# MatteoBattilana/CUDAVideoStream

Measured on AMD Instinct MI355X. Metric: 1920×1080 RGB24 frames/sec (diff+threshold+pack); achieved HBM GB/s vs peak, higher is better.
Workload: dtype u8

## Files before the change

### cudavideostream_amd/csrc/core.hip

```cpp
#include <cmath>
#include <cstdio>
#include <cstdlib>
#include <cstring>
#include <new>
#include <string>
#include <vector>

#include "../../include/mi355diff.h"
#include "cwire_common.h"

using namespace mi355;

static inline size_t code_chunks(size_t max_batch) { return (max_batch + 2) / 3 + 1; }

namespace {

thread_local std::string g_err;

int fail(int code, const char *what, hipError_t e = hipSuccess) {
    char buf[512];
    if (e != hipSuccess)
        snprintf(buf, sizeof buf, "%s: %s (%s)", what, hipGetErrorName(e), hipGetErrorString(e));
    else
        snprintf(buf, sizeof buf, "%s", what);
    g_err = buf;
    return code;
}

// ... 2 lines not shown
        hipError_t _e = (expr);                                   \
        if (_e != hipSuccess) return fail(MI355_ERR_HIP, #expr, _e); \
    } while (0)

}

struct mi355_core {
    mi355_config cfg{};
    int device = 0;
    uint32_t n = 0;
    uint32_t ntiles = 0;
    hipStream_t own_stream = nullptr;
    hipStream_t stream = nullptr;

    uint8_t *state = nullptr, *in = nullptr, *aux = nullptr, *vis = nullptr;
    uint4 *rec = nullptr, *meta = nullptr;
    uint32_t *codes = nullptr;
    uint32_t *groff = nullptr, *totals = nullptr;
    uint64_t scan_epoch = 0;
    uint32_t *offsets = nullptr;
    int32_t *one_xs = nullptr;
    uint8_t *one_diff = nullptr;
    int32_t *hist = nullptr, *thr = nullptr;
    uint32_t *red_bounds = nullptr;
    uint32_t *cw_cnt = nullptr;
    uint4 *cw_items = nullptr;
    uint32_t *cw_esc = nullptr;
    CwaFrame *cwa_ftab = nullptr;
    uint4 *cwa_chunk = nullptr;
    uint4 *cwa_dir = nullptr;
    uint8_t *gray1 = nullptr;
// ... 11 lines not shown

    static constexpr int kMaxSlots = 8;
    struct Slot {
        uint8_t *d_in = nullptr, *d_vis = nullptr;
        uint32_t *h_count = nullptr;
        hipEvent_t uploaded = nullptr, painted = nullptr, packed = nullptr, shown = nullptr;
        bool has_vis = false;
        int64_t ticket = -1;
    };
    Slot slots[kMaxSlots];
    int nslots = 0;
    int64_t next_ticket = 0;
    hipStream_t up_stream = nullptr, down_stream = nullptr;

    struct LogSet {
        uint4 *rec = nullptr, *meta = nullptr;
        uint32_t *codes = nullptr, *groff = nullptr, *totals = nullptr;
        hipEvent_t packed = nullptr, expanded = nullptr;
        bool in_use = false;
    };
    static constexpr int kSets = 2;
    LogSet set[kSets];
    int flip = 0;
    hipStream_t side = nullptr;
    hipEvent_t side_done = nullptr;
    bool pipeline_ok = true;
    int median_rows = 0;
    uint32_t cu_count = 0;
    hipStream_t main2 = nullptr;
    hipEvent_t packed2[kSets] = {};
    static constexpr uint32_t kDensePct = 40;
// ... 116 lines not shown
}

int need_red_bounds(mi355_core *c) {
    if (c->red_bounds || c->n == 0) return MI355_OK;
    return dev_alloc(c, &c->red_bounds, (size_t)c->cfg.max_batch * red_bounds_per_frame(c->n));
}

int setup_pipeline(mi355_core *c) {
    if (c->side || !c->pipeline_ok) return MI355_OK;
    const size_t T = (size_t)c->cfg.max_batch, W = c->ntiles;
    mi355_core::LogSet &s0 = c->set[0], &s1 = c->set[1];
    s0.rec = c->rec; s0.codes = c->codes; s0.meta = c->meta; s0.groff = c->groff; s0.totals = c->totals;
    bool ok = true;
    ok = ok && hipMalloc((void **)&s1.rec, T * W * 1024) == hipSuccess;
    ok = ok && hipMalloc((void **)&s1.codes, code_chunks(T) * W * 1024) == hipSuccess;
    ok = ok && hipMalloc((void **)&s1.meta, T * W * 16) == hipSuccess;
    ok = ok && hipMalloc((void **)&s1.groff, T * expand_groups(c->ntiles) * 16) == hipSuccess;
    ok = ok && hipMalloc((void **)&s1.totals, (2 * T + 2) * sizeof(uint32_t)) == hipSuccess;
    ok = ok && hipMemsetAsync(s1.totals, 0, (2 * T + 2) * sizeof(uint32_t), c->stream) == hipSuccess &&
         hipStreamSynchronize(c->stream) == hipSuccess;
    ok = ok && make_stream(c, &c->side) == hipSuccess;
    ok = ok && make_stream(c, &c->main2) == hipSuccess;
    for (int i = 0; i < mi355_core::kSets && ok; i++) {
        const unsigned flags = hipEventDisableTiming | hipEventReleaseToDevice;
        ok = hipEventCreateWithFlags(&c->set[i].packed, flags) == hipSuccess &&
             hipEventCreateWithFlags(&c->set[i].expanded, flags) == hipSuccess &&
             hipEventCreateWithFlags(&c->packed2[i], flags) == hipSuccess &&
             hipEventCreateWithFlags(&c->fork[i], flags) == hipSuccess;
    }
    if (!ok) {
        (void)hipGetLastError();
        void *ptrs[] = {s1.rec, s1.codes, s1.meta, s1.groff, s1.totals};
        for (void *p : ptrs) if (p) (void)hipFree(p);
        s1.rec = nullptr; s1.meta = nullptr; s1.codes = s1.groff = s1.totals = nullptr;
        if (c->side) { (void)hipStreamDestroy(c->side); c->side = nullptr; }
        if (c->main2) { (void)hipStreamDestroy(c->main2); c->main2 = nullptr; }
        for (int i = 0; i < mi355_core::kSets; i++) {
            hipEvent_t *evs[] = {&c->set[i].packed, &c->set[i].expanded, &c->packed2[i], &c->fork[i]};
            for (hipEvent_t *e : evs) if (*e) { (void)hipEventDestroy(*e); *e = nullptr; }
        }
        c->pipeline_ok = false;
        return MI355_OK;
    }
    c->workspace += T * W * 1024 + code_chunks(T) * W * 1024 + T * W * 16 + T * expand_groups(c->ntiles) * 16 + (2 * T + 2) * 4;
    return MI355_OK;
}

struct CwireOut {
    uint64_t *frame_pos;
    uint8_t *cwire;
    uint64_t capacity;
};

CwireDirectArgs cwire_args(mi355_core *c, const CwireOut *cw, const uint32_t *d_offsets, uint32_t ntiles) {
    CwireDirectArgs x{};
    x.x.offsets = d_offsets;
    x.x.ntiles = ntiles;
    x.items = c->cw_items;
    x.esc = c->cw_esc;
// ... 54 lines not shown
    a.cur = (const uint8_t *)d_cur;
    a.prev = (const uint8_t *)d_prev;
    a.state = c->state;
    a.stride = stride;
    a.n = c->n;
    a.nframes = nframes;
    a.thr = c->cfg.threshold;
    a.ntiles = c->ntiles;
    a.tile_begin = 0;
    a.tile_end = c->ntiles;
    a.rec = ls.rec;
    a.codes = ls.codes;
    a.codes_bytes = (uint32_t)(code_chunks((size_t)c->cfg.max_batch) * c->ntiles * 1024u);
    a.meta = ls.meta;
    a.rec_bytes = (uint32_t)((size_t)c->cfg.max_batch * c->ntiles * 1024u);
    a.meta_bytes = (uint32_t)((size_t)c->cfg.max_batch * c->ntiles * 16u);
    const bool aligned = (((uintptr_t)d_cur | (uintptr_t)d_prev | stride) & 15u) == 0 && 3 * (uint64_t)stride + c->n < (1ull << 32);
    bool pair_once = false;
    if (pair) {
        const int64_t d = (int64_t)((intptr_t)d_prev - (intptr_t)d_cur), st = (int64_t)stride, T = nframes;
        bool shared = false;
        const int64_t k0 = d / st;
        for (int64_t k = k0 - 1; k <= k0 + 1; k++)
            if (k > -T && k < T && (d - k * st < 0 ? k * st - d : d - k * st) < (int64_t)c->n) shared = true;
        pair_once = !shared;
    }
    const uint32_t k1_blocks = 4u * c->cu_count;
    const bool split = pipelined && c->main2 && c->ntiles >= 64;
    if (split) {
        const uint32_t cut = (c->ntiles / 2) & ~3u;
        uint32_t blocks0 = 0, blocks1 = 0;
// ... 81 lines not shown
    if (!cfg || !out) return fail(MI355_ERR_INVALID, "null argument");
    *out = nullptr;
    if (cfg->width < 0 || cfg->height < 0) return fail(MI355_ERR_INVALID, "negative frame size");
    if (cfg->threshold < 0 || cfg->threshold > 255) return fail(MI355_ERR_INVALID, "threshold outside 0..255");
    if (cfg->max_batch < 1) return fail(MI355_ERR_INVALID, "max_batch < 1");
    if (cfg->visualizer < 0 || cfg->visualizer > 5) return fail(MI355_ERR_INVALID, "unknown visualizer");
    if (cfg->flags & ~MI355_FLAG_OWN_QUEUES) return fail(MI355_ERR_INVALID, "flags: unknown bit (MI355_FLAG_OWN_QUEUES is the only flag of this version of the library)");
    const uint64_t n64 = 3ull * (uint64_t)cfg->width * (uint64_t)cfg->height;
    if (n64 >= (1ull << 31)) return fail(MI355_ERR_INVALID, "frame larger than 2 GiB");
    {
        const uint64_t tiles = (n64 + kTileBytes - 1) / kTileBytes, mb = (uint64_t)cfg->max_batch;
        const uint64_t chunks = mb > code_chunks((size_t)mb) ? mb : (uint64_t)code_chunks((size_t)mb);
        if (tiles * kTileBytes * chunks >= (1ull << 32))
            return fail(MI355_ERR_INVALID, "max_batch * frame bytes must stay below 2^32");
    }

    int ndev = 0;
    hipError_t e = hipGetDeviceCount(&ndev);
    if (e != hipSuccess || ndev <= 0)
        return fail(MI355_ERR_HIP, "no HIP device available (libmi355diff has no CPU fallback)", e);
    mi355_core *c = new (std::nothrow) mi355_core;
    if (!c) return fail(MI355_ERR_INVALID, "out of host memory");
    c->cfg = *cfg;
    if (const char *v = getenv("MI355_PIPELINE")) c->pipeline_ok = v[0] != '0';
    if (cfg->device >= 0) c->device = cfg->device;
    else if ((e = hipGetDevice(&c->device)) != hipSuccess) { delete c; return fail(MI355_ERR_HIP, "hipGetDevice", e); }
    if (c->device >= ndev) { delete c; return fail(MI355_ERR_INVALID, "device ordinal out of range"); }

    c->n = (uint32_t)n64;
    c->ntiles = (c->n + kTileBytes - 1) / kTileBytes;
// ... 2 lines not shown
        if (hipGetDeviceProperties(&prop, c->device) == hipSuccess && prop.multiProcessorCount > 0) c->cu_count = (uint32_t)prop.multiProcessorCount;
    }
    const size_t T = (size_t)cfg->max_batch, W = c->ntiles, N = c->n;

    int rc = use_device(c);
    if (!rc) { e = make_stream(c, &c->own_stream); if (e != hipSuccess) rc = fail(MI355_ERR_HIP, "hipStreamCreate", e); }
    c->stream = c->own_stream;
    for (int i = 0; i < mi355_core::kEvRing * mi355_core::kEvPer && !rc; i++) { e = hipEventCreateWithFlags(&c->ev[i / mi355_core::kEvPer][i % mi355_core::kEvPer], hipEventDisableSystemFence); if (e != hipSuccess) rc = fail(MI355_ERR_HIP, "hipEventCreate", e); }
    if (!rc && (e = init_gray_table()) != hipSuccess) rc = fail(MI355_ERR_HIP, "init_gray_table", e);
    if (!rc) rc = dev_alloc(c, &c->state, N + 16);
    if (!rc) rc = dev_alloc(c, &c->in, N + 16);
    if (!rc) rc = dev_alloc(c, &c->aux, N + 16);
    if (!rc) rc = dev_alloc(c, &c->vis, N + 16);
    if (!rc) rc = dev_alloc(c, &c->rec, T * W * 64);
    if (!rc) rc = dev_alloc(c, &c->codes, code_chunks(T) * W * 256);
    if (!rc) rc = dev_alloc(c, &c->meta, T * W);
    if (!rc) rc = dev_alloc(c, &c->groff, T * expand_groups(c->ntiles) * 4);
    if (!rc) rc = dev_alloc(c, &c->totals, 2 * T + 2);
    if (!rc) { e = hipMemsetAsync(c->totals, 0, (2 * T + 2) * sizeof(uint32_t), c->own_stream); if (e != hipSuccess) rc = fail(MI355_ERR_HIP, "hipMemset", e); }
    if (!rc) rc = dev_alloc(c, &c->offsets, T + 1);
    if (!rc) rc = dev_alloc(c, &c->cw_cnt, (size_t)kCwireSlots);
    if (!rc) rc = dev_alloc(c, &c->cw_items, T * cwire_items_per_frame(c->ntiles));
    if (!rc) rc = dev_alloc(c, &c->cw_esc, T);
    if (!rc) rc = dev_alloc(c, &c->cwa_ftab, T);
    if (!rc) rc = dev_alloc(c, &c->cwa_chunk, T * cwa_chunks(c->n));
    if (!rc) rc = dev_alloc(c, &c->cwa_dir, T * cwa_tiles(c->n));
    if (!rc) rc = dev_alloc(c, &c->one_xs, N + 4);
    if (!rc) rc = dev_alloc(c, &c->one_diff, N + 16);
    if (!rc) rc = dev_alloc(c, &c->hist, 256 * T);
    if (!rc) rc = dev_alloc(c, &c->thr, T);
    if (!rc) rc = dev_alloc(c, &c->k9, 9);
// ... 985 lines not shown
```

### cudavideostream_amd/csrc/diff_pack.hip

```cpp
#include <cstdio>
#include <vector>

#include "cwire_common.h"
#include "pack_common.h"

namespace mi355 {

constexpr int kStreamPrefetch = 4;
template <bool PAIR>
struct PrefetchOf { static constexpr int value = PAIR ? 2 : kStreamPrefetch; };
static_assert(kStreamPrefetch % 2 == 0, "frames are processed in pairs");

typedef uint32_t u32x4 __attribute__((ext_vector_type(4)));
constexpr uint32_t kRsrcWord3 = 0x00020000u;
constexpr uint32_t kOOB = 0xFFFFFFFFu;

__device__ __forceinline__ __amdgpu_buffer_rsrc_t make_rsrc(const void *p, uint32_t bytes) {
    return __builtin_amdgcn_make_buffer_rsrc(const_cast<void *>(p), 0, (int)bytes, (int)kRsrcWord3);
}

struct LogOut {
    __amdgpu_buffer_rsrc_t codes, recs, meta;
};

template <bool HIGH>
__device__ __forceinline__ void compare_step(const uint4 c, uint4 &s, ThrConst tc, uint32_t (&dm)[4], uint32_t &m16) {
    const uint32_t cw[4] = {c.x, c.y, c.z, c.w};
    uint32_t sw[4] = {s.x, s.y, s.z, s.w};
// ... 1 lines not shown
#pragma unroll
    for (int k = 0; k < 4; k++) {
        uint32_t x;
        fh[k] = dword_flags<HIGH>(cw[k], sw[k], tc, x);
        const uint32_t mask = __builtin_amdgcn_perm(0u, 0u, fh[k]);
        dm[k] = bytes_sub_from_x(cw[k], sw[k], x, tc.h) & mask;
        sw[k] = bitop3<(TA & TC) | (TB & ~TC)>(cw[k], sw[k], mask);
    }
    s = make_uint4(sw[0], sw[1], sw[2], sw[3]);
    const uint32_t lo = __builtin_amdgcn_udot4(fh[1], tc.w1, __builtin_amdgcn_udot4(fh[0], tc.w0, 0u, false), false);
    const uint32_t hi = __builtin_amdgcn_udot4(fh[3], tc.w1, __builtin_amdgcn_udot4(fh[2], tc.w0, 0u, false), false);
    m16 = (lo + (hi << 8)) >> 7;
}

struct LogPos {
    uint32_t ptrC, roomC, ptrM, roomM;
};

__device__ __forceinline__ uint32_t emit_step(const uint32_t (&dm)[4], uint32_t m16, const LogOut &lg, LogPos &lp,
                                              uint32_t jump, uint32_t lane24, uint32_t &pc, uint32_t &pm) {
    const bool cand = m16 != 0u;
    const bool multi = (m16 & (m16 - 1u)) != 0u;
    const uint64_t bc = __ballot(cand), bm = __ballot(multi);
    const uint32_t rankC = __builtin_amdgcn_mbcnt_hi((uint32_t)(bc >> 32), __builtin_amdgcn_mbcnt_lo((uint32_t)bc, 0u));
    const uint32_t rankM = __builtin_amdgcn_mbcnt_hi((uint32_t)(bm >> 32), __builtin_amdgcn_mbcnt_lo((uint32_t)bm, 0u));
    const uint32_t nc = (uint32_t)__builtin_popcountll(bc), nm = (uint32_t)__builtin_popcountll(bm);
    pc = lp.ptrC;
    pm = lp.ptrM;
    if (nc == 0u) return 0u;
    if (nm > lp.roomM) { lp.ptrM += lp.roomM * 16u + jump; lp.roomM = 64u; }
    pm = lp.ptrM;
    if (nm == 64u) {
        const u32x4 v = {dm[0], dm[1], dm[2], dm[3]};
        __builtin_amdgcn_raw_buffer_store_b128(v, lg.recs, pm + rankM * 16u, 0, 0);
        lp.ptrM += 64u * 16u;
        lp.roomM -= 64u;
        return 64u | (64u << 16);
    }
    if (nc > lp.roomC) { lp.ptrC += lp.roomC * 4u + jump; lp.roomC = 256u; }
    pc = lp.ptrC;
    const uint32_t one = __builtin_amdgcn_sad_u8((dm[0] | dm[1]) | (dm[2] | dm[3]), 0u, 0u);
    const uint32_t code = m16 | ((multi ? rankM : one) << 16) | lane24;
    __builtin_amdgcn_raw_buffer_store_b32(code, lg.codes, cand ? pc + rankC * 4u : kOOB, 0, 0);
    const u32x4 v = {dm[0], dm[1], dm[2], dm[3]};
    __builtin_amdgcn_raw_buffer_store_b128(v, lg.recs, multi ? pm + rankM * 16u : kOOB, 0, 0);
    lp.ptrC += nc * 4u;
    lp.roomC -= nc;
    lp.ptrM += nm * 16u;
    lp.roomM -= nm;
    return nc | (nm << 16);
}

template <bool PAIR, bool FAST>
struct Group {
    static constexpr int kPrefetch = PrefetchOf<PAIR>::value;
    uint4 c[kPrefetch];
    uint4 p[kPrefetch];

    template <bool ONCE>
    __device__ __forceinline__ void load_desc(__amdgpu_buffer_rsrc_t cur, __amdgpu_buffer_rsrc_t prev, const uint32_t (&voff)[kPrefetch]) {
#pragma unroll
        for (int d = 0; d < kPrefetch; d++) {
            const u32x4 v = __builtin_amdgcn_raw_buffer_load_b128(cur, voff[d], 0, ONCE ? 2 : 0);
            c[d] = make_uint4(v.x, v.y, v.z, v.w);
            if (PAIR) {
// ... 11 lines not shown
            const bool in = t0 + d <= last;
            const uint8_t *cb = uniform_ptr(in ? cur0 + (size_t)d * a.stride : cur_last);
            c[d] = load16<FAST, !PAIR>(cb + byte_off, valid);
            if (PAIR) {
                const uint8_t *pb = uniform_ptr(in ? prev0 + (size_t)d * a.stride : prev_last);
                p[d] = load16<FAST>(pb + byte_off, valid);
            }
        }
    }
};

template <bool PAIR, bool FAST, bool HIGH>
__device__ __forceinline__ void pack_group(const PackArgs &a, const Group<PAIR, FAST> &g, int t0, uint4 &st,
                                           LogPos &lp, uint32_t tile, ThrConst tc, int lane, const LogOut &lg) {
    constexpr int kPrefetch = PrefetchOf<PAIR>::value;
    uint4 meta = make_uint4(0, 0, 0, 0);
    const uint32_t lane24 = ((uint32_t)lane << 24) | (tile << 30);
    const uint32_t jump = (a.ntiles - 1u) * 1024u;
#pragma unroll
    for (int d = 0; d < kPrefetch; d += 2) {
        const int t = t0 + d;
        if (t >= a.nframes) break;
        const bool two = t + 1 < a.nframes;
        uint32_t dm0[4], m0, m1 = 0, pc0, pm0, pc1 = 0, pm1 = 0;
        if (PAIR) st = g.p[d];
        compare_step<HIGH>(g.c[d], st, tc, dm0, m0);
        const uint32_t c0 = emit_step(dm0, m0, lg, lp, jump, lane24, pc0, pm0);
        uint32_t c1 = 0;
        if (two) {
            if (PAIR) st = g.p[d + 1];
            uint32_t dm1[4];
            compare_step<HIGH>(g.c[d + 1], st, tc, dm1, m1);
            c1 = emit_step(dm1, m1, lg, lp, jump, lane24, pc1, pm1);
        }
        const uint32_t both = (uint32_t)__builtin_popcount(m0) | ((uint32_t)__builtin_popcount(m1) << 16);
        const uint32_t tot = (uint32_t)__builtin_amdgcn_readlane(wave_inclusive_scan((int)both), 63);
        write_lane(meta.x, pc0, d);
        write_lane(meta.y, pm0, d);
        write_lane(meta.z, tot & 0xffffu, d);
        write_lane(meta.w, c0, d);
        write_lane(meta.x, pc1, d + 1);
        write_lane(meta.y, pm1, d + 1);
        write_lane(meta.z, tot >> 16, d + 1);
        write_lane(meta.w, c1, d + 1);
    }
    const uint32_t moff = (__umul24((uint32_t)t0 + (uint32_t)lane, a.ntiles) + tile) * 16u;
    const u32x4 mv = {meta.x, meta.y, meta.z, meta.w};
    __builtin_amdgcn_raw_buffer_store_b128(mv, lg.meta, (lane < kPrefetch && t0 + lane < a.nframes) ? moff : kOOB, 0, 0);
}

template <bool PAIR, bool FAST, bool HIGH, bool ONCE>
__device__ __forceinline__ void pack_tile(const PackArgs &a, uint32_t tile, uint32_t byte_off,
                                          int valid, int lane) {
    const int T = a.nframes;
    const ThrConst tc = make_thr((uint32_t)a.thr);
    const LogOut lg{make_rsrc(a.codes, a.codes_bytes), make_rsrc(a.rec, a.rec_bytes), make_rsrc(a.meta, a.meta_bytes)};

    uint4 st = make_uint4(0, 0, 0, 0);
    if (!PAIR) st = load16<FAST>(a.state + byte_off, valid);

    Group<PAIR, FAST> ga, gb;
    LogPos lp{tile * 1024u, 256u, tile * 1024u, 64u};
    constexpr int kPrefetch = PrefetchOf<PAIR>::value;
    const size_t gstep = (size_t)kPrefetch * a.stride;
    if (FAST) {
        uint32_t voff[kPrefetch];
#pragma unroll
        for (int d = 0; d < kPrefetch; d++) voff[d] = byte_off + (uint32_t)d * (uint32_t)a.stride;
        const uint8_t *cb = a.cur, *pb = a.prev;
        int64_t left = (int64_t)(T - 1) * (int64_t)a.stride + (int64_t)a.n;
        auto desc = [&](const uint8_t *base) {
            const uint32_t bytes = left <= 0 ? 0u : (left > 0xffffffffll ? 0xffffffffu : (uint32_t)left);
            return make_rsrc(base, bytes);
        };
        ga.template load_desc<ONCE>(desc(cb), desc(pb), voff);
        for (int t0 = 0;;) {
            cb += gstep; if (PAIR) pb += gstep; left -= (int64_t)gstep;
// ... 87 lines not shown
        for (int w = 0; w < NW; w++) {
            const uint32_t x = lds[w];
            lds[w] = acc;
            acc += x;
        }
        lds[NW] = acc;
    }
    __syncthreads();
    const uint32_t r = lds[wave] + incl - v;
    block_total = lds[NW];
    __syncthreads();
    return r;
}

constexpr uint32_t kXTiles = 64;
constexpr uint32_t kScanChunk = 1024;
constexpr uint32_t kScanDepth = 24;

__device__ __forceinline__ void publish_total(uint64_t *slot, uint32_t total, uint64_t epoch) {
    __hip_atomic_store(slot, (uint64_t)total | (epoch << kTotalBits), __ATOMIC_RELAXED, __HIP_MEMORY_SCOPE_AGENT);
}
__device__ __forceinline__ uint32_t read_total(const uint64_t *slot, uint64_t epoch) {
    uint64_t v;
    do v = __hip_atomic_load(slot, __ATOMIC_RELAXED, __HIP_MEMORY_SCOPE_AGENT);
    while ((v >> kTotalBits) != epoch);
    return (uint32_t)v & ((1u << kTotalBits) - 1u);
}

__global__ __launch_bounds__(256) void k_scan_groups(const uint4 *meta, uint32_t *roff, uint64_t *totals,
                                                     uint32_t ntiles, uint32_t ngroups, uint32_t *ticket,
                                                     uint64_t epoch, uint32_t *offsets, uint64_t *note) {
    static_assert(kXTiles == 64, "one wave reduces one group");
    __builtin_amdgcn_s_setprio(3);
    __shared__ uint32_t s_sum[kScanChunk];
    __shared__ uint32_t s_part[kScanChunk][3];
    __shared__ uint32_t s_scan[5];
    const uint32_t lane = threadIdx.x & 63, wave = threadIdx.x >> 6;
    const size_t row = (size_t)blockIdx.x * ntiles;
    uint32_t *out = roff + (size_t)blockIdx.x * ngroups * 4u;
    uint32_t carry = 0;
    for (uint32_t g0 = 0; g0 < ngroups; g0 += kScanChunk) {
        const uint32_t gn = min(kScanChunk, ngroups - g0);
        for (uint32_t g = wave * kScanDepth; g < gn; g += 4u * kScanDepth) {
            uint32_t z[kScanDepth];
#pragma unroll
            for (uint32_t k = 0; k < kScanDepth; k++) {
                const uint32_t tile = (g0 + g + k) * kXTiles + lane;
                z[k] = meta[row + min(tile, ntiles - 1u)].z;
            }
#pragma unroll
            for (uint32_t k = 0; k < kScanDepth; k++) {
                const uint32_t tile = (g0 + g + k) * kXTiles + lane;
                if (g + k >= gn || tile >= ntiles) z[k] = 0u;
                const uint32_t incl = (uint32_t)wave_inclusive_scan((int)z[k]);
                if (g + k < gn) {
                    if (lane == 63) s_sum[g + k] = incl;
                    if ((lane & 15u) == 15u && lane < 48u) s_part[g + k][lane >> 4] = incl;
                }
            }
        }
        __syncthreads();
        uint32_t v[4], sum = 0;
#pragma unroll
        for (uint32_t i = 0; i < 4; i++) {
            const uint32_t idx = threadIdx.x * 4 + i;
            v[i] = idx < gn ? s_sum[idx] : 0u;
            sum += v[i];
        }
        uint32_t total;
        uint32_t acc = carry + block_exclusive_scan<4>(sum, s_scan, total);
#pragma unroll
        for (uint32_t i = 0; i < 4; i++) {
            const uint32_t idx = threadIdx.x * 4 + i;
            if (idx < gn)
                *reinterpret_cast<uint4 *>(out + 4 * (size_t)(g0 + idx)) =
                    make_uint4(acc, acc + s_part[idx][0], acc + s_part[idx][1], acc + s_part[idx][2]);
            acc += v[i];
        }
        carry += total;
        __syncthreads();
    }
    __shared__ uint32_t s_is_last;
    if (threadIdx.x == 0) {
        publish_total(&totals[blockIdx.x], carry, epoch);
        s_is_last = __hip_atomic_fetch_add(ticket, 1u, __ATOMIC_RELAXED, __HIP_MEMORY_SCOPE_AGENT) == gridDim.x - 1;
    }
    __syncthreads();
    if (!s_is_last) return;
    const uint32_t nframes = gridDim.x;
    carry = 0;
    for (uint32_t base = 0; base < nframes; base += 256) {
        const uint32_t t = base + threadIdx.x;
        const uint32_t v = t < nframes ? read_total(&totals[t], epoch) : 0u;
        uint32_t total;
        const uint32_t ex = block_exclusive_scan<4>(v, s_scan, total);
        if (t < nframes) offsets[t] = carry + ex;
        carry += total;
    }
    if (threadIdx.x == 0) {
        offsets[nframes] = carry;
        __hip_atomic_store(ticket, 0u, __ATOMIC_RELAXED, __HIP_MEMORY_SCOPE_AGENT);
        if (note) __hip_atomic_store(note, (uint64_t)carry | ((uint64_t)nframes << 32), __ATOMIC_RELAXED, __HIP_MEMORY_SCOPE_SYSTEM);
    }
}

uint32_t expand_groups(uint32_t ntiles) { return (ntiles + kXTiles - 1) / kXTiles; }

hipError_t launch_scan(const uint4 *meta, uint32_t *roff, uint64_t *totals, uint32_t ntiles,
                       int nframes, uint32_t *offsets, uint32_t *ticket, uint64_t epoch, uint64_t *note, hipStream_t s) {
    hipLaunchKernelGGL(k_scan_groups, dim3(nframes), dim3(256), 0, s, meta, roff, totals, ntiles,
                       expand_groups(ntiles), ticket, epoch, offsets, note);
    return hipGetLastError();
}

__device__ __forceinline__ void store_u32_unaligned(uint8_t *p, uint32_t v) { __builtin_memcpy(p, &v, 4); }

__device__ __forceinline__ void lds_handoff() {
    __builtin_amdgcn_fence(__ATOMIC_ACQ_REL, "wavefront");
    __builtin_amdgcn_wave_barrier();
}

typedef uint32_t u32x4a4 __attribute__((ext_vector_type(4), aligned(4)));
typedef uint32_t u32x4a1 __attribute__((ext_vector_type(4), aligned(1)));
typedef uint32_t u32a1 __attribute__((aligned(1)));
template <bool BYTE_ALIGNED>
__device__ __forceinline__ void store_out4(uint8_t *p, uint32_t x, uint32_t y, uint32_t z, uint32_t w) {
// ... 31 lines not shown
    }
    const uint32_t tail = 4u * n4 + lane;
    if (tail < n) {
        const uint32_t v = stage[tail];
        store_u32_unaligned(xsp + 4 * (size_t)tail, xs0 + (v >> 8));
        dfp[tail] = (uint8_t)v;
    }
}

constexpr uint32_t kWTiles = 16;
constexpr uint32_t kWStage = 1024;
constexpr uint32_t kFList = 128;
constexpr uint32_t kFStage = kWStage;
constexpr uint32_t kXLight = 4;
constexpr int kXHeavyMax = 12;

__device__ __forceinline__ int row_inclusive_scan(int v) {
    v = dpp_add<0x111, 0xf>(v);
    v = dpp_add<0x112, 0xf>(v);
    v = dpp_add<0x114, 0xf>(v);
    v = dpp_add<0x118, 0xf>(v);
    return v;
}

__device__ __forceinline__ void walk_records(uint32_t m16, uint32_t e, uint32_t src16, uint4 rec, uint32_t *stage, uint32_t lane) {
    const uint32_t cnt = (uint32_t)__builtin_popcount(m16);
    const uint64_t heavy = __ballot(cnt > kXLight);
    if (__builtin_popcountll(heavy) > kXHeavyMax) {
        const uint32_t w[4] = {rec.x, rec.y, rec.z, rec.w};
        const uint32_t base = src16 << 8;
// ... 198 lines not shown
    }
    lds_handoff();
    sink.flush(stage, flushed, carry - flushed, xs0);
}

template <bool WIRE>
__global__ __launch_bounds__(64) __attribute__((amdgpu_waves_per_eu(8, 8))) void k_expand(const ExpandArgs a) {
    __shared__ __attribute__((aligned(16))) uint2 s_list[kFList];
    __shared__ __attribute__((aligned(16))) uint32_t s_stage[kWStage];
    __builtin_amdgcn_s_setprio(2);
    const uint32_t lane = threadIdx.x & 63u;
    asm volatile("v_mov_b32 v63, 0" ::: "v63");
    const uint32_t t = blockIdx.y, sub = blockIdx.x;
    if (sub * kWTiles >= a.ntiles) return;
    const uint32_t ngroups = (a.ntiles + kXTiles - 1) / kXTiles;
    const uint32_t tile = sub * kWTiles + lane;
    const __amdgpu_buffer_rsrc_t metas = make_rsrc(a.meta + (size_t)t * a.ntiles, a.ntiles * 16u);
    const u32x4 mq = __builtin_amdgcn_raw_buffer_load_b128(metas, lane < kWTiles ? tile * 16u : kOOB, 0, 0);
    typedef const __attribute__((address_space(4))) uint32_t *cptr;
    const cptr offs_c = (cptr)(uintptr_t)a.offsets, roff_c = (cptr)(uintptr_t)a.roff;
    const uint32_t off_t = offs_c[t];
    const uint32_t roff = roff_c[(size_t)t * ngroups * 4u + sub];
    const uint32_t n_t = WIRE ? offs_c[t + 1] - off_t : 0u;
    asm volatile("" ::"s"(off_t), "s"(roff), "s"(n_t));
    const uint4 m = make_uint4(mq.x, mq.y, mq.z, mq.w);
    size_t head = 0;
    if (WIRE) {
        head = 4 * (size_t)t + 5 * (size_t)off_t;
        if (sub == 0 && lane == 0 && head + 4 <= a.capacity) store_u32_unaligned(a.wire + head, n_t);
    }
    const uint32_t nc = m.w & 0xffffu;
    const uint32_t both = m.z | (m.w & 0xffff0000u);
    const uint32_t bincl = (uint32_t)row_inclusive_scan((int)both);
// ... 34 lines not shown
    const uint32_t gx = (a.ntiles + kWTiles - 1) / kWTiles;
    const dim3 grid((gx + 7u) / 8u * 8u, nframes);
    if (a.wire)
        hipLaunchKernelGGL(k_expand<true>, grid, dim3(64), 0, s, a);
    else
        hipLaunchKernelGGL(k_expand<false>, grid, dim3(64), 0, s, a);
    return hipGetLastError();
}

__host__ __device__ uint32_t cwire_items_per_frame(uint32_t ntiles) { return (ntiles + kWTiles - 1) / kWTiles; }

__global__ __launch_bounds__(64) void k_cwire_items(const CwireDirectArgs a) {
    const uint32_t lane = threadIdx.x & 63u;
    const uint32_t t = blockIdx.y, sub = blockIdx.x, ntiles = a.x.ntiles;
    if (sub * kWTiles >= ntiles) return;
    const __amdgpu_buffer_rsrc_t metas = make_rsrc(a.x.meta + (size_t)t * ntiles, ntiles * 16u);
    const u32x4 m = __builtin_amdgcn_raw_buffer_load_b128(metas, lane < kWTiles ? (sub * kWTiles + lane) * 16u : kOOB, 0, 0);
    const __amdgpu_buffer_rsrc_t codes = make_rsrc(a.x.codes, a.x.codes_bytes), recs = make_rsrc(a.x.rec, a.x.rec_bytes);
    uint32_t code[kWTiles];
#pragma unroll
    for (uint32_t i = 0; i < kWTiles; i++) {
        const uint32_t cx = (uint32_t)__builtin_amdgcn_readlane((int)m.x, i), cw = (uint32_t)__builtin_amdgcn_readlane((int)m.w, i);
        const bool load = (cw >> 16) != 64u && lane < (cw & 0xffffu);
        code[i] = __builtin_amdgcn_raw_buffer_load_b32(codes, load ? cx + 4u * lane : kOOB, 0, 0);
    }
    uint32_t first = 0, end = 0, esc = 0, nent = 0;
#pragma unroll
    for (uint32_t i = 0; i < kWTiles; i++) {
        const uint32_t cw = (uint32_t)__builtin_amdgcn_readlane((int)m.w, i), nc = cw & 0xffffu;
        if (nc == 0u) continue;
        nent += (uint32_t)__builtin_amdgcn_readlane((int)m.z, i);
        const uint32_t base = (sub * kWTiles + i) * kTileBytes;
// ... 128 lines not shown
    CwireCursor &cur;
    __device__ __forceinline__ void flush(const uint32_t *stage, uint32_t, uint32_t count, uint32_t xs0) { flush_cwire(stage, count, xs0, cur); }
};

__global__ __launch_bounds__(64) __attribute__((amdgpu_waves_per_eu(8, 8))) void k_expand_cwire(const CwireDirectArgs a) {
    __shared__ __attribute__((aligned(16))) uint4 s_tinfo[kWTiles];
    __shared__ __attribute__((aligned(16))) uint32_t s_stage[kWStage];
    __builtin_amdgcn_s_setprio(2);
    const uint32_t lane = threadIdx.x & 63u;
    const uint32_t t = blockIdx.y, sub = blockIdx.x, ntiles = a.x.ntiles;
    if (sub * kWTiles >= ntiles) return;
    const uint64_t p0 = a.frame_pos[t], p1 = a.frame_pos[t + 1];
    if (p1 > a.capacity) return;
    const uint4 item = a.items[(size_t)t * cwire_items_per_frame(ntiles) + sub];
    if (item.w == 0u) return;
    const __amdgpu_buffer_rsrc_t metas = make_rsrc(a.x.meta + (size_t)t * ntiles, ntiles * 16u);
    const u32x4 mq = __builtin_amdgcn_raw_buffer_load_b128(metas, lane < kWTiles ? (sub * kWTiles + lane) * 16u : kOOB, 0, 0);
    const uint32_t ngroups = (ntiles + kXTiles - 1) / kXTiles;
    const uint32_t off_t = a.x.offsets[t], n = a.x.offsets[t + 1] - off_t;
    const uint32_t e = cwire_record_escapes(p1 - p0, n);
    CwireCursor cur{CwireSections<uint8_t>(a.cwire, p0, n, e), n, e, 0u, 0u, 0u};
    cur.entry = a.x.roff[(size_t)t * ngroups * 4u + sub];
    cur.end = item.y;
    cur.erank = item.z;
    if (lane < kWTiles) s_tinfo[lane] = make_uint4(mq.x, mq.y, mq.z, mq.w);
    lds_handoff();
    const uint32_t xs0 = sub * kWTiles * kTileBytes;
    CwireSink sink{cur};
    expand_tiles(a.x, s_tinfo, s_stage, lane, xs0, sink);
}

hipError_t launch_expand_cwire(const CwireDirectArgs &a, int nframes, hipStream_t s) {
// ... 15 lines not shown
```

### cudavideostream_amd/csrc/internal.h

```cpp
#ifndef MI355_INTERNAL_H_
#define MI355_INTERNAL_H_

#include <hip/hip_runtime.h>
#include <stddef.h>
#include <stdint.h>

namespace mi355 {

constexpr uint32_t kTileBytes = 1024;
constexpr uint32_t kWavesPerBlock = 4;

struct PackArgs {
    const uint8_t *cur;
    const uint8_t *prev;
    uint8_t *state;
    size_t stride;
    uint32_t n;
    int32_t nframes;
    int32_t thr;
    uint32_t ntiles;
    uint32_t tile_begin;
    uint32_t tile_end;
    uint32_t *codes;
    uint4 *rec;
    uint4 *meta;
    uint32_t codes_bytes;
    uint32_t rec_bytes;
    uint32_t meta_bytes;
};

struct ExpandArgs {
    const uint32_t *codes;
    const uint4 *rec;
    const uint4 *meta;
    const uint32_t *roff;
    const uint32_t *offsets;
    uint32_t ntiles;
    uint32_t codes_bytes;
    uint32_t rec_bytes;
    int32_t *out_xs;
    uint8_t *out_diff;
    uint8_t *wire;
    size_t capacity;
};

}
struct mi355_core;
namespace mi355 {
int set_error(int code, const char *what);
hipStream_t core_stream(::mi355_core *c);
int core_device(const ::mi355_core *c);

hipError_t launch_diff_pack(const PackArgs &a, bool pair, bool aligned, bool pair_once ,
                            uint32_t max_blocks , hipStream_t s);
uint32_t expand_groups(uint32_t ntiles);
constexpr int kTotalBits = 31;
constexpr uint64_t kEpochWrap = 1ull << (64 - kTotalBits);
inline bool next_scan_epoch(uint64_t &epoch) {
    if (++epoch < kEpochWrap) return false;
    epoch = 1;
    return true;
}
hipError_t launch_scan(const uint4 *meta, uint32_t *roff, uint64_t *totals , uint32_t ntiles,
                       int nframes, uint32_t *offsets, uint32_t *ticket ,
                       uint64_t epoch ,
                       uint64_t *note , hipStream_t s);
hipError_t launch_expand(const ExpandArgs &a, int nframes, hipStream_t s);
__host__ __device__ uint32_t cwire_items_per_frame(uint32_t ntiles);
struct CwireDirectArgs {
    ExpandArgs x;
    uint4 *items;
    uint32_t *esc;
    uint64_t *frame_pos;
    uint8_t *cwire;
    uint64_t capacity;
};
hipError_t launch_expand_cwire(const CwireDirectArgs &a, int nframes, hipStream_t s);

// ... 105 lines not shown
```

### cudavideostream_amd/csrc/pack_common.h

```cpp
#ifndef MI355_PACK_COMMON_H_
#define MI355_PACK_COMMON_H_

#include "internal.h"

namespace mi355 {

template <int CTRL, int ROW_MASK>
__device__ __forceinline__ int dpp_add(int v) {
    return v + __builtin_amdgcn_update_dpp(0, v, CTRL, ROW_MASK, 0xf, false);
}

__device__ __forceinline__ int wave_inclusive_scan(int v) {
    v = dpp_add<0x111, 0xf>(v);
    v = dpp_add<0x112, 0xf>(v);
    v = dpp_add<0x114, 0xf>(v);
    v = dpp_add<0x118, 0xf>(v);
    v = dpp_add<0x142, 0xa>(v);
    v = dpp_add<0x143, 0xc>(v);
    return v;
}

template <int CTRL, int ROW_MASK>
__device__ __forceinline__ uint32_t dpp_max(uint32_t v) {
    const uint32_t o = (uint32_t)__builtin_amdgcn_update_dpp(0, (int)v, CTRL, ROW_MASK, 0xf, false);
// ... 95 lines not shown
    return (const uint8_t *)(((uint64_t)hi << 32) | lo);
}

__device__ __forceinline__ uint32_t nonzero_bytes(uint32_t v) {
    return (((v & kL) + kL) | v) & kH;
}

__device__ __forceinline__ uint32_t record_map16(uint4 rec) {
    const uint32_t g0 = __builtin_amdgcn_udot4(nonzero_bytes(rec.x), 0x08040201u, 0u, false);
    const uint32_t g1 = __builtin_amdgcn_udot4(nonzero_bytes(rec.y), 0x08040201u, 0u, false);
    const uint32_t g2 = __builtin_amdgcn_udot4(nonzero_bytes(rec.z), 0x08040201u, 0u, false);
    const uint32_t g3 = __builtin_amdgcn_udot4(nonzero_bytes(rec.w), 0x08040201u, 0u, false);
    return (g0 + (g1 << 4) + (g2 << 8) + (g3 << 12)) >> 7;
}

}
#endif
```

### include/mi355diff.h

```cpp
#ifndef MI355DIFF_H_
#define MI355DIFF_H_

#include <stddef.h>
#include <stdint.h>

#ifdef __cplusplus
extern "C" {
#endif

#define MI355_OK 0
#define MI355_ERR_INVALID (-1)
#define MI355_ERR_HIP (-2)
#define MI355_ERR_STATE (-3)

#define MI355_VIS_NONE 0
#define MI355_VIS_HEAT 1
#define MI355_VIS_RED 2
#define MI355_VIS_RED_OVERLAP 3
#define MI355_VIS_GRAY 4
#define MI355_VIS_BINARIZE 5

typedef struct mi355_core mi355_core;

typedef struct mi355_config {
    int32_t width;
    int32_t height;
    int32_t threshold;
    int32_t max_batch;
    int32_t device;
    int32_t noise_filter;
    int32_t visualizer;
    int32_t flags;
} mi355_config;
#define MI355_FLAG_OWN_QUEUES 1

#define MI355_ABI_VERSION 10
int mi355_abi_version(void);

int mi355_create(const mi355_config *cfg, mi355_core **out);
void mi355_destroy(mi355_core *core);
const char *mi355_last_error(void);
size_t mi355_frame_bytes(const mi355_core *core);
size_t mi355_workspace_bytes(const mi355_core *core);
#define MI355_PREPARE_BATCHES 1u
#define MI355_PREPARE_GRAY_CHAIN 2u
#define MI355_PREPARE_RED_CLEAR 4u
#define MI355_PREPARE_CONV_KXK 8u
#define MI355_PREPARE_EXEC 16u
#define MI355_PREPARE_ALL 31u
int mi355_prepare(mi355_core *core, unsigned what);

// ... 132 lines not shown
```

Measured before the change: 552,400.

## Compress per-tile meta to 8 bytes with interleaved frame layout and batched scan

```diff
diff --git a/cudavideostream_amd/csrc/core.hip b/cudavideostream_amd/csrc/core.hip
--- a/cudavideostream_amd/csrc/core.hip
+++ b/cudavideostream_amd/csrc/core.hip
@@ -8,10 +8,13 @@
 
 #include "../../include/mi355diff.h"
 #include "cwire_common.h"
+#include "pack_common.h"
 
 using namespace mi355;
 
 static inline size_t code_chunks(size_t max_batch) { return (max_batch + 2) / 3 + 1; }
+static_assert(MI355_MAX_BATCH == kMetaMaxBatch, "the header states the meta word's limit");
+static_assert((MI355_MAX_BATCH + 2) / 3 + 1 < (1 << 13), "13 bits of the meta word hold every code chunk");
 
 namespace {
 
@@ -44,7 +47,7 @@
     hipStream_t stream = nullptr;
 
     uint8_t *state = nullptr, *in = nullptr, *aux = nullptr, *vis = nullptr;
-    uint4 *rec = nullptr, *meta = nullptr;
+    uint4 *rec = nullptr; uint2 *meta = nullptr;
     uint32_t *codes = nullptr;
     uint32_t *groff = nullptr, *totals = nullptr;
     uint64_t scan_epoch = 0;
@@ -86,7 +89,7 @@
     hipStream_t up_stream = nullptr, down_stream = nullptr;
 
     struct LogSet {
-        uint4 *rec = nullptr, *meta = nullptr;
+        uint4 *rec = nullptr; uint2 *meta = nullptr;
         uint32_t *codes = nullptr, *groff = nullptr, *totals = nullptr;
         hipEvent_t packed = nullptr, expanded = nullptr;
         bool in_use = false;
@@ -233,7 +236,7 @@
     bool ok = true;
     ok = ok && hipMalloc((void **)&s1.rec, T * W * 1024) == hipSuccess;
     ok = ok && hipMalloc((void **)&s1.codes, code_chunks(T) * W * 1024) == hipSuccess;
-    ok = ok && hipMalloc((void **)&s1.meta, T * W * 16) == hipSuccess;
+    ok = ok && hipMalloc((void **)&s1.meta, meta_words(T, W) * 8) == hipSuccess;
     ok = ok && hipMalloc((void **)&s1.groff, T * expand_groups(c->ntiles) * 16) == hipSuccess;
     ok = ok && hipMalloc((void **)&s1.totals, (2 * T + 2) * sizeof(uint32_t)) == hipSuccess;
     ok = ok && hipMemsetAsync(s1.totals, 0, (2 * T + 2) * sizeof(uint32_t), c->stream) == hipSuccess &&
@@ -261,7 +264,7 @@
         c->pipeline_ok = false;
         return MI355_OK;
     }
-    c->workspace += T * W * 1024 + code_chunks(T) * W * 1024 + T * W * 16 + T * expand_groups(c->ntiles) * 16 + (2 * T + 2) * 4;
+    c->workspace += T * W * 1024 + code_chunks(T) * W * 1024 + meta_words(T, W) * 8 + T * expand_groups(c->ntiles) * 16 + (2 * T + 2) * 4;
     return MI355_OK;
 }
 
@@ -346,7 +349,7 @@
     a.codes_bytes = (uint32_t)(code_chunks((size_t)c->cfg.max_batch) * c->ntiles * 1024u);
     a.meta = ls.meta;
     a.rec_bytes = (uint32_t)((size_t)c->cfg.max_batch * c->ntiles * 1024u);
-    a.meta_bytes = (uint32_t)((size_t)c->cfg.max_batch * c->ntiles * 16u);
+    a.meta_bytes = (uint32_t)(meta_words((size_t)c->cfg.max_batch, c->ntiles) * 8u);
     const bool aligned = (((uintptr_t)d_cur | (uintptr_t)d_prev | stride) & 15u) == 0 && 3 * (uint64_t)stride + c->n < (1ull << 32);
     bool pair_once = false;
     if (pair) {
@@ -458,6 +461,7 @@
         if (tiles * kTileBytes * chunks >= (1ull << 32))
             return fail(MI355_ERR_INVALID, "max_batch * frame bytes must stay below 2^32");
     }
+    if ((uint32_t)cfg->max_batch > kMetaMaxBatch) return fail(MI355_ERR_INVALID, "max_batch above 4096 (MI355_MAX_BATCH)");
 
     int ndev = 0;
     hipError_t e = hipGetDeviceCount(&ndev);
@@ -490,7 +494,7 @@
     if (!rc) rc = dev_alloc(c, &c->vis, N + 16);
     if (!rc) rc = dev_alloc(c, &c->rec, T * W * 64);
     if (!rc) rc = dev_alloc(c, &c->codes, code_chunks(T) * W * 256);
-    if (!rc) rc = dev_alloc(c, &c->meta, T * W);
+    if (!rc) rc = dev_alloc(c, &c->meta, meta_words(T, W));
     if (!rc) rc = dev_alloc(c, &c->groff, T * expand_groups(c->ntiles) * 4);
     if (!rc) rc = dev_alloc(c, &c->totals, 2 * T + 2);
     if (!rc) { e = hipMemsetAsync(c->totals, 0, (2 * T + 2) * sizeof(uint32_t), c->own_stream); if (e != hipSuccess) rc = fail(MI355_ERR_HIP, "hipMemset", e); }
diff --git a/cudavideostream_amd/csrc/diff_pack.hip b/cudavideostream_amd/csrc/diff_pack.hip
--- a/cudavideostream_amd/csrc/diff_pack.hip
+++ b/cudavideostream_amd/csrc/diff_pack.hip
@@ -12,6 +12,7 @@
 static_assert(kStreamPrefetch % 2 == 0, "frames are processed in pairs");
 
 typedef uint32_t u32x4 __attribute__((ext_vector_type(4)));
+typedef uint32_t u32x2 __attribute__((ext_vector_type(2)));
 constexpr uint32_t kRsrcWord3 = 0x00020000u;
 constexpr uint32_t kOOB = 0xFFFFFFFFu;
 
@@ -43,31 +44,34 @@
 }
 
 struct LogPos {
-    uint32_t ptrC, roomC, ptrM, roomM;
+    uint32_t ptrC, roomC, posC, ptrM, roomM, posM;
 };
 
 __device__ __forceinline__ uint32_t emit_step(const uint32_t (&dm)[4], uint32_t m16, const LogOut &lg, LogPos &lp,
-                                              uint32_t jump, uint32_t lane24, uint32_t &pc, uint32_t &pm) {
+                                              uint32_t jump, uint32_t lane24, uint32_t &lo) {
+    uint32_t pc, pm;
     const bool cand = m16 != 0u;
     const bool multi = (m16 & (m16 - 1u)) != 0u;
     const uint64_t bc = __ballot(cand), bm = __ballot(multi);
     const uint32_t rankC = __builtin_amdgcn_mbcnt_hi((uint32_t)(bc >> 32), __builtin_amdgcn_mbcnt_lo((uint32_t)bc, 0u));
     const uint32_t rankM = __builtin_amdgcn_mbcnt_hi((uint32_t)(bm >> 32), __builtin_amdgcn_mbcnt_lo((uint32_t)bm, 0u));
     const uint32_t nc = (uint32_t)__builtin_popcountll(bc), nm = (uint32_t)__builtin_popcountll(bm);
-    pc = lp.ptrC;
+    lo = 0u;
+    if (nc == 0u) return 0u;
+    if (nm > lp.roomM) { lp.ptrM += lp.roomM * 16u + jump; lp.posM += lp.roomM; lp.roomM = 64u; }
     pm = lp.ptrM;
-    if (nc == 0u) return 0u;
-    if (nm > lp.roomM) { lp.ptrM += lp.roomM * 16u + jump; lp.roomM = 64u; }
-    pm = lp.ptrM;
+    const uint32_t pos_m = lp.posM;
     if (nm == 64u) {
         const u32x4 v = {dm[0], dm[1], dm[2], dm[3]};
         __builtin_amdgcn_raw_buffer_store_b128(v, lg.recs, pm + rankM * 16u, 0, 0);
         lp.ptrM += 64u * 16u;
         lp.roomM -= 64u;
-        return 64u | (64u << 16);
-    }
-    if (nc > lp.roomC) { lp.ptrC += lp.roomC * 4u + jump; lp.roomC = 256u; }
+        lp.posM += 64u;
+        return meta_pack_hi(64u, 64u, pos_m);
+    }
+    if (nc > lp.roomC) { lp.ptrC += lp.roomC * 4u + jump; lp.posC += lp.roomC; lp.roomC = 256u; }
     pc = lp.ptrC;
+    lo = meta_pack_lo(0u, lp.posC);
     const uint32_t one = __builtin_amdgcn_sad_u8((dm[0] | dm[1]) | (dm[2] | dm[3]), 0u, 0u);
     const uint32_t code = m16 | ((multi ? rankM : one) << 16) | lane24;
     __builtin_amdgcn_raw_buffer_store_b32(code, lg.codes, cand ? pc + rankC * 4u : kOOB, 0, 0);
@@ -75,9 +79,11 @@
     __builtin_amdgcn_raw_buffer_store_b128(v, lg.recs, multi ? pm + rankM * 16u : kOOB, 0, 0);
     lp.ptrC += nc * 4u;
     lp.roomC -= nc;
+    lp.posC += nc;
     lp.ptrM += nm * 16u;
     lp.roomM -= nm;
-    return nc | (nm << 16);
+    lp.posM += nm;
+    return meta_pack_hi(nc, nm, pos_m);
 }
 
 template <bool PAIR, bool FAST>
@@ -119,7 +125,7 @@
 __device__ __forceinline__ void pack_group(const PackArgs &a, const Group<PAIR, FAST> &g, int t0, uint4 &st,
                                            LogPos &lp, uint32_t tile, ThrConst tc, int lane, const LogOut &lg) {
     constexpr int kPrefetch = PrefetchOf<PAIR>::value;
-    uint4 meta = make_uint4(0, 0, 0, 0);
+    uint32_t mlo = 0, mhi = 0;
     const uint32_t lane24 = ((uint32_t)lane << 24) | (tile << 30);
     const uint32_t jump = (a.ntiles - 1u) * 1024u;
 #pragma unroll
@@ -127,31 +133,27 @@
         const int t = t0 + d;
         if (t >= a.nframes) break;
         const bool two = t + 1 < a.nframes;
-        uint32_t dm0[4], m0, m1 = 0, pc0, pm0, pc1 = 0, pm1 = 0;
+        uint32_t dm0[4], m0, m1 = 0, lo0, lo1 = 0;
         if (PAIR) st = g.p[d];
         compare_step<HIGH>(g.c[d], st, tc, dm0, m0);
-        const uint32_t c0 = emit_step(dm0, m0, lg, lp, jump, lane24, pc0, pm0);
+        const uint32_t c0 = emit_step(dm0, m0, lg, lp, jump, lane24, lo0);
         uint32_t c1 = 0;
         if (two) {
             if (PAIR) st = g.p[d + 1];
             uint32_t dm1[4];
             compare_step<HIGH>(g.c[d + 1], st, tc, dm1, m1);
-            c1 = emit_step(dm1, m1, lg, lp, jump, lane24, pc1, pm1);
+            c1 = emit_step(dm1, m1, lg, lp, jump, lane24, lo1);
         }
         const uint32_t both = (uint32_t)__builtin_popcount(m0) | ((uint32_t)__builtin_popcount(m1) << 16);
         const uint32_t tot = (uint32_t)__builtin_amdgcn_readlane(wave_inclusive_scan((int)both), 63);
-        write_lane(meta.x, pc0, d);
-        write_lane(meta.y, pm0, d);
-        write_lane(meta.z, tot & 0xffffu, d);
-        write_lane(meta.w, c0, d);
-        write_lane(meta.x, pc1, d + 1);
-        write_lane(meta.y, pm1, d + 1);
-        write_lane(meta.z, tot >> 16, d + 1);
-        write_lane(meta.w, c1, d + 1);
-    }
-    const uint32_t moff = (__umul24((uint32_t)t0 + (uint32_t)lane, a.ntiles) + tile) * 16u;
-    const u32x4 mv = {meta.x, meta.y, meta.z, meta.w};
-    __builtin_amdgcn_raw_buffer_store_b128(mv, lg.meta, (lane < kPrefetch && t0 + lane < a.nframes) ? moff : kOOB, 0, 0);
+        write_lane(mlo, lo0 | (tot & 0xffffu), d);
+        write_lane(mhi, c0, d);
+        write_lane(mlo, lo1 | (tot >> 16), d + 1);
+        write_lane(mhi, c1, d + 1);
+    }
+    const uint32_t moff = (((uint32_t)t0 >> 2) * a.ntiles + tile) * 32u + (((uint32_t)t0 & 3u) + (uint32_t)lane) * 8u;
+    const u32x2 mv = {mlo, mhi};
+    __builtin_amdgcn_raw_buffer_store_b64(mv, lg.meta, (lane < kPrefetch && t0 + lane < a.nframes) ? moff : kOOB, 0, 0);
 }
 
 template <bool PAIR, bool FAST, bool HIGH, bool ONCE>
@@ -165,7 +167,7 @@
     if (!PAIR) st = load16<FAST>(a.state + byte_off, valid);
 
     Group<PAIR, FAST> ga, gb;
-    LogPos lp{tile * 1024u, 256u, tile * 1024u, 64u};
+    LogPos lp{tile * 1024u, 256u, 0u, tile * 1024u, 64u, 0u};
     constexpr int kPrefetch = PrefetchOf<PAIR>::value;
     const size_t gstep = (size_t)kPrefetch * a.stride;
     if (FAST) {
@@ -283,7 +285,7 @@
 }
 
 constexpr uint32_t kXTiles = 64;
-constexpr uint32_t kScanChunk = 1024;
+constexpr uint32_t kScanChunk = 512;
 constexpr uint32_t kScanDepth = 24;
 
 __device__ __forceinline__ void publish_total(uint64_t *slot, uint32_t total, uint64_t epoch) {
@@ -296,67 +298,79 @@
     return (uint32_t)v & ((1u << kTotalBits) - 1u);
 }
 
-__global__ __launch_bounds__(256) void k_scan_groups(const uint4 *meta, uint32_t *roff, uint64_t *totals,
-                                                     uint32_t ntiles, uint32_t ngroups, uint32_t *ticket,
+__global__ __launch_bounds__(256) void k_scan_groups(const uint2 *meta, uint32_t *roff, uint64_t *totals,
+                                                     uint32_t ntiles, uint32_t ngroups, uint32_t nframes, uint32_t *ticket,
                                                      uint64_t epoch, uint32_t *offsets, uint64_t *note) {
     static_assert(kXTiles == 64, "one wave reduces one group");
+    static_assert(kScanChunk == 64 * 8, "a wave scans a frame's group sums eight to a lane");
     __builtin_amdgcn_s_setprio(3);
-    __shared__ uint32_t s_sum[kScanChunk];
-    __shared__ uint32_t s_part[kScanChunk][3];
+    __shared__ uint32_t s_sum[4][kScanChunk];
+    __shared__ uint32_t s_part[4][kScanChunk][3];
     __shared__ uint32_t s_scan[5];
+    __shared__ uint32_t s_tot[4];
     const uint32_t lane = threadIdx.x & 63, wave = threadIdx.x >> 6;
-    const size_t row = (size_t)blockIdx.x * ntiles;
-    uint32_t *out = roff + (size_t)blockIdx.x * ngroups * 4u;
+    const uint32_t t0 = blockIdx.x * 4u;
+    const uint32_t live = min(4u, nframes - t0);
+    const uint4 *row = reinterpret_cast<const uint4 *>(meta + (size_t)blockIdx.x * ntiles * 4u);
+    uint32_t *out = roff + (size_t)(t0 + wave) * ngroups * 4u;
     uint32_t carry = 0;
     for (uint32_t g0 = 0; g0 < ngroups; g0 += kScanChunk) {
         const uint32_t gn = min(kScanChunk, ngroups - g0);
         for (uint32_t g = wave * kScanDepth; g < gn; g += 4u * kScanDepth) {
-            uint32_t z[kScanDepth];
+            uint4 q[kScanDepth][2];
+#pragma unroll
+            for (uint32_t k = 0; k < kScanDepth; k++) {
+                const uint32_t tile = min((g0 + g + k) * kXTiles + lane, ntiles - 1u);
+                q[k][0] = row[2u * (size_t)tile];
+                q[k][1] = row[2u * (size_t)tile + 1u];
+            }
 #pragma unroll
             for (uint32_t k = 0; k < kScanDepth; k++) {
                 const uint32_t tile = (g0 + g + k) * kXTiles + lane;
-                z[k] = meta[row + min(tile, ntiles - 1u)].z;
-            }
-#pragma unroll
-            for (uint32_t k = 0; k < kScanDepth; k++) {
-                const uint32_t tile = (g0 + g + k) * kXTiles + lane;
-                if (g + k >= gn || tile >= ntiles) z[k] = 0u;
-                const uint32_t incl = (uint32_t)wave_inclusive_scan((int)z[k]);
-                if (g + k < gn) {
-                    if (lane == 63) s_sum[g + k] = incl;
-                    if ((lane & 15u) == 15u && lane < 48u) s_part[g + k][lane >> 4] = incl;
+                const bool in = g + k < gn && tile < ntiles;
+                const uint32_t z[4] = {q[k][0].x, q[k][0].z, q[k][1].x, q[k][1].z};
+#pragma unroll
+                for (uint32_t f = 0; f < 4; f++) {
+                    const uint32_t incl = (uint32_t)wave_inclusive_scan(in && f < live ? (int)meta_bytes_of(z[f]) : 0);
+                    if (g + k < gn) {
+                        if (lane == 63) s_sum[f][g + k] = incl;
+                        if ((lane & 15u) == 15u && lane < 48u) s_part[f][g + k][lane >> 4] = incl;
+                    }
                 }
             }
         }
         __syncthreads();
-        uint32_t v[4], sum = 0;
-#pragma unroll
-        for (uint32_t i = 0; i < 4; i++) {
-            const uint32_t idx = threadIdx.x * 4 + i;
-            v[i] = idx < gn ? s_sum[idx] : 0u;
+        uint32_t v[8], sum = 0;
+#pragma unroll
+        for (uint32_t i = 0; i < 8; i++) {
+            const uint32_t idx = lane * 8 + i;
+            v[i] = idx < gn ? s_sum[wave][idx] : 0u;
             sum += v[i];
         }
-        uint32_t total;
-        uint32_t acc = carry + block_exclusive_scan<4>(sum, s_scan, total);
-#pragma unroll
-        for (uint32_t i = 0; i < 4; i++) {
-            const uint32_t idx = threadIdx.x * 4 + i;
-            if (idx < gn)
-                *reinterpret_cast<uint4 *>(out + 4 * (size_t)(g0 + idx)) =
-                    make_uint4(acc, acc + s_part[idx][0], acc + s_part[idx][1], acc + s_part[idx][2]);
-            acc += v[i];
-        }
-        carry += total;
+        const uint32_t incl = (uint32_t)wave_inclusive_scan((int)sum);
+        uint32_t acc = carry + incl - sum;
+        if (wave < live) {
+#pragma unroll
+            for (uint32_t i = 0; i < 8; i++) {
+                const uint32_t idx = lane * 8 + i;
+                if (idx < gn)
+                    *reinterpret_cast<uint4 *>(out + 4 * (size_t)(g0 + idx)) =
+                        make_uint4(acc, acc + s_part[wave][idx][0], acc + s_part[wave][idx][1], acc + s_part[wave][idx][2]);
+                acc += v[i];
+            }
+        }
+        carry += (uint32_t)__builtin_amdgcn_readlane((int)incl, 63);
         __syncthreads();
     }
     __shared__ uint32_t s_is_last;
+    if (lane == 0) s_tot[wave] = carry;
+    __syncthreads();
     if (threadIdx.x == 0) {
-        publish_total(&totals[blockIdx.x], carry, epoch);
+        for (uint32_t f = 0; f < live; f++) publish_total(&totals[t0 + f], s_tot[f], epoch);
         s_is_last = __hip_atomic_fetch_add(ticket, 1u, __ATOMIC_RELAXED, __HIP_MEMORY_SCOPE_AGENT) == gridDim.x - 1;
     }
     __syncthreads();
     if (!s_is_last) return;
-    const uint32_t nframes = gridDim.x;
     carry = 0;
     for (uint32_t base = 0; base < nframes; base += 256) {
         const uint32_t t = base + threadIdx.x;
@@ -375,10 +389,10 @@
 
 uint32_t expand_groups(uint32_t ntiles) { return (ntiles + kXTiles - 1) / kXTiles; }
 
-hipError_t launch_scan(const uint4 *meta, uint32_t *roff, uint64_t *totals, uint32_t ntiles,
+hipError_t launch_scan(const uint2 *meta, uint32_t *roff, uint64_t *totals, uint32_t ntiles,
                        int nframes, uint32_t *offsets, uint32_t *ticket, uint64_t epoch, uint64_t *note, hipStream_t s) {
-    hipLaunchKernelGGL(k_scan_groups, dim3(nframes), dim3(256), 0, s, meta, roff, totals, ntiles,
-                       expand_groups(ntiles), ticket, epoch, offsets, note);
+    hipLaunchKernelGGL(k_scan_groups, dim3(((uint32_t)nframes + 3u) / 4u), dim3(256), 0, s, meta, roff, totals, ntiles,
+                       expand_groups(ntiles), (uint32_t)nframes, ticket, epoch, offsets, note);
     return hipGetLastError();
 }
 
@@ -440,6 +454,15 @@
 constexpr uint32_t kFStage = kWStage;
 constexpr uint32_t kXLight = 4;
 constexpr int kXHeavyMax = 12;
+
+__device__ __forceinline__ uint4 load_item_meta(const uint2 *meta, uint32_t ntiles, uint32_t t, uint32_t sub, uint32_t lane) {
+    const uint32_t tile = sub * kWTiles + lane;
+    const bool live = lane < kWTiles && tile < ntiles;
+    const __amdgpu_buffer_rsrc_t metas = make_rsrc(meta + (size_t)(t >> 2) * ntiles * 4u, ntiles * 32u);
+    const u32x2 w = __builtin_amdgcn_raw_buffer_load_b64(metas, live ? tile * 32u + (t & 3u) * 8u : kOOB, 0, 0);
+    return make_uint4(live ? meta_code_offset(w.x, ntiles, tile) : 0u, live ? meta_rec_offset(w.y, ntiles, tile) : 0u,
+                      meta_bytes_of(w.x), meta_cand_of(w.y) | (meta_multi_of(w.y) << 16));
+}
 
 __device__ __forceinline__ int row_inclusive_scan(int v) {
     v = dpp_add<0x111, 0xf>(v);
@@ -668,9 +691,7 @@
     const uint32_t t = blockIdx.y, sub = blockIdx.x;
     if (sub * kWTiles >= a.ntiles) return;
     const uint32_t ngroups = (a.ntiles + kXTiles - 1) / kXTiles;
-    const uint32_t tile = sub * kWTiles + lane;
-    const __amdgpu_buffer_rsrc_t metas = make_rsrc(a.meta + (size_t)t * a.ntiles, a.ntiles * 16u);
-    const u32x4 mq = __builtin_amdgcn_raw_buffer_load_b128(metas, lane < kWTiles ? tile * 16u : kOOB, 0, 0);
+    const uint4 mq = load_item_meta(a.meta, a.ntiles, t, sub, lane);
     typedef const __attribute__((address_space(4))) uint32_t *cptr;
     const cptr offs_c = (cptr)(uintptr_t)a.offsets, roff_c = (cptr)(uintptr_t)a.roff;
     const uint32_t off_t = offs_c[t];
@@ -735,8 +756,7 @@
     const uint32_t lane = threadIdx.x & 63u;
     const uint32_t t = blockIdx.y, sub = blockIdx.x, ntiles = a.x.ntiles;
     if (sub * kWTiles >= ntiles) return;
-    const __amdgpu_buffer_rsrc_t metas = make_rsrc(a.x.meta + (size_t)t * ntiles, ntiles * 16u);
-    const u32x4 m = __builtin_amdgcn_raw_buffer_load_b128(metas, lane < kWTiles ? (sub * kWTiles + lane) * 16u : kOOB, 0, 0);
+    const uint4 m = load_item_meta(a.x.meta, ntiles, t, sub, lane);
     const __amdgpu_buffer_rsrc_t codes = make_rsrc(a.x.codes, a.x.codes_bytes), recs = make_rsrc(a.x.rec, a.x.rec_bytes);
     uint32_t code[kWTiles];
 #pragma unroll
@@ -895,8 +915,7 @@
     if (p1 > a.capacity) return;
     const uint4 item = a.items[(size_t)t * cwire_items_per_frame(ntiles) + sub];
     if (item.w == 0u) return;
-    const __amdgpu_buffer_rsrc_t metas = make_rsrc(a.x.meta + (size_t)t * ntiles, ntiles * 16u);
-    const u32x4 mq = __builtin_amdgcn_raw_buffer_load_b128(metas, lane < kWTiles ? (sub * kWTiles + lane) * 16u : kOOB, 0, 0);
+    const uint4 mq = load_item_meta(a.x.meta, ntiles, t, sub, lane);
     const uint32_t ngroups = (ntiles + kXTiles - 1) / kXTiles;
     const uint32_t off_t = a.x.offsets[t], n = a.x.offsets[t + 1] - off_t;
     const uint32_t e = cwire_record_escapes(p1 - p0, n);
diff --git a/cudavideostream_amd/csrc/internal.h b/cudavideostream_amd/csrc/internal.h
--- a/cudavideostream_amd/csrc/internal.h
+++ b/cudavideostream_amd/csrc/internal.h
@@ -23,7 +23,7 @@
     uint32_t tile_end;
     uint32_t *codes;
     uint4 *rec;
-    uint4 *meta;
+    uint2 *meta;
     uint32_t codes_bytes;
     uint32_t rec_bytes;
     uint32_t meta_bytes;
@@ -32,7 +32,7 @@
 struct ExpandArgs {
     const uint32_t *codes;
     const uint4 *rec;
-    const uint4 *meta;
+    const uint2 *meta;
     const uint32_t *roff;
     const uint32_t *offsets;
     uint32_t ntiles;
@@ -61,7 +61,7 @@
     epoch = 1;
     return true;
 }
-hipError_t launch_scan(const uint4 *meta, uint32_t *roff, uint64_t *totals , uint32_t ntiles,
+hipError_t launch_scan(const uint2 *meta, uint32_t *roff, uint64_t *totals , uint32_t ntiles,
                        int nframes, uint32_t *offsets, uint32_t *ticket ,
                        uint64_t epoch ,
                        uint64_t *note , hipStream_t s);
diff --git a/cudavideostream_amd/csrc/pack_common.h b/cudavideostream_amd/csrc/pack_common.h
--- a/cudavideostream_amd/csrc/pack_common.h
+++ b/cudavideostream_amd/csrc/pack_common.h
@@ -4,6 +4,29 @@
 #include "internal.h"
 
 namespace mi355 {
+
+constexpr uint32_t kMetaMaxBatch = 1u << 12;
+constexpr uint32_t kMetaBytesMask = 0x7ffu;
+
+__host__ __device__ inline uint32_t meta_pack_lo(uint32_t bytes, uint32_t code_pos) { return bytes | (code_pos << 11); }
+__host__ __device__ inline uint32_t meta_pack_hi(uint32_t cand, uint32_t multi, uint32_t rec_pos) { return cand | (multi << 7) | (rec_pos << 14); }
+__host__ __device__ inline uint32_t meta_bytes_of(uint32_t lo) { return lo & kMetaBytesMask; }
+__host__ __device__ inline uint32_t meta_cand_of(uint32_t hi) { return hi & 127u; }
+__host__ __device__ inline uint32_t meta_multi_of(uint32_t hi) { return (hi >> 7) & 127u; }
+__host__ __device__ inline uint32_t meta_code_offset(uint32_t lo, uint32_t ntiles, uint32_t tile) {
+    const uint32_t pos = lo >> 11;
+    return ((pos >> 8) * ntiles + tile) * 1024u + (pos & 255u) * 4u;
+}
+__host__ __device__ inline uint32_t meta_rec_offset(uint32_t hi, uint32_t ntiles, uint32_t tile) {
+    const uint32_t pos = hi >> 14;
+    return ((pos >> 6) * ntiles + tile) * 1024u + (pos & 63u) * 16u;
+}
+__host__ __device__ inline size_t meta_index(uint32_t t, uint32_t ntiles, uint32_t tile) {
+    return ((size_t)(t >> 2) * ntiles + tile) * 4u + (t & 3u);
+}
+__host__ __device__ inline size_t meta_words(size_t T, size_t ntiles) { return (T + 3) / 4 * 4 * ntiles; }
+
+#if defined(__HIPCC__)
 
 template <int CTRL, int ROW_MASK>
 __device__ __forceinline__ int dpp_add(int v) {
@@ -133,5 +156,7 @@
     return (g0 + (g1 << 4) + (g2 << 8) + (g3 << 12)) >> 7;
 }
 
+#endif
+
 }
 #endif
diff --git a/include/mi355diff.h b/include/mi355diff.h
--- a/include/mi355diff.h
+++ b/include/mi355diff.h
@@ -35,6 +35,7 @@
 #define MI355_FLAG_OWN_QUEUES 1
 
 #define MI355_ABI_VERSION 10
+#define MI355_MAX_BATCH 4096
 int mi355_abi_version(void);
 
 int mi355_create(const mi355_config *cfg, mi355_core **out);
```

After: 563,500, median of 6. +2.0%, better.
